# karfly/learnable-triangulation-pytorch

Hardware: AMD Instinct MI355X
Metric: multi-view samples/sec (4-view vol-softmax forward) (higher is better)
Workload: dtype bf16; 1 GPU; BASELINE config 2: volumetric-softmax forward, 4 views 384x384, 64^3 voxel cube, ResNet-152, random-init weights; per_gpu_batch=64, global_batch=64, parallelism=batch-sharded replicas x1, no data-path collective, hip_graph=True, self_launched=False

## Files before the change

include/lt_hip.h:

```cpp
#ifndef LT_HIP_H
#define LT_HIP_H

#include <stddef.h>
#include <stdint.h>

#ifdef __cplusplus
extern "C" {
#endif

#define LT_ABI_VERSION 1

enum { LT_F32 = 0, LT_BF16 = 1,
       LT_FP8 = 2  };
enum { LT_OK = 0, LT_ERR_INVALID = -1, LT_ERR_UNSUPPORTED = -2, LT_ERR_LAUNCH = -3 };

enum { LT_AGG_SUM = 0, LT_AGG_MAX = 1, LT_AGG_SOFTMAX = 2, LT_AGG_CONF = 3,
       LT_AGG_CONF_NORM = 4  };

enum {
    LT_EPI_RELU_PRE = 1,
    LT_EPI_RELU_POST = 2,
    LT_EPI_STORE_F32 = 4,
    LT_EPI_SIGMOID = 8,
    LT_EPI_RES_F32 = 64,
// ... 21 lines not shown
    int32_t dtype;
    int32_t N, D, H, W, Cin;
    int32_t Do, Ho, Wo;
    int32_t stride[3], pad[3];
    int32_t OD, OH, OW;
    int32_t out_stride[3];
    int32_t Cout, ldc;
    int32_t cout_pad, k_pad;
    int32_t nphase;
    int32_t flags;
    int32_t tile;
    int32_t stages;
    lt_conv_phase phase[LT_CONV_MAX_PHASES];
} lt_conv_desc;

int lt_conv_pack_weights(const void* weight, int32_t cout_pad, int32_t k_pad, void* packed, void* stream);
int lt_conv_pack_weights_t32(const void* weight, int32_t cout_pad, int32_t k_pad, int32_t cin, int32_t ntaps, void* packed,
                             void* stream);
int lt_conv_pack_weights32(const void* weight, int32_t cout_pad, int32_t k_pad, void* packed, void* stream);

enum { LT_TILE_AUTO = 0,
       LT_TILE_128x128 = 1, LT_TILE_128x64 = 2, LT_TILE_256x32 = 3, LT_TILE_256x16 = 4, LT_TILE_64x64 = 5,
       LT_TILE2_128x128 = 11, LT_TILE2_128x64 = 12, LT_TILE2_256x32 = 13, LT_TILE2_256x16 = 14, LT_TILE2_64x64 = 15,
       LT_TILE_HALO = 20,
       LT_TILE3_288 = 30,
       LT_TILE_DIRECT = 99  };

int lt_conv_fwd(const lt_conv_desc* desc, const void* x, const float* bias, const float* scale, const float* shift,
                const void* residual, void* y, void* stream);
typedef struct lt_conv_skip {
    const void* x;
    int32_t cin;
    const void* weight_frag;
} lt_conv_skip;
int lt_conv_skip_fwd(const lt_conv_desc* desc, const void* x, const float* bias, const float* scale, const float* shift,
                     const lt_conv_skip* skip, void* y, void* stream);
typedef struct lt_conv_cat2 {
    const void* x;
    int32_t cin, H, W, stride;
} lt_conv_cat2;
int lt_conv_cat2_fwd(const lt_conv_desc* desc, const void* x, const lt_conv_cat2* second, const float* bias, const float* scale, const float* shift,
                     const void* residual, void* y, void* stream);
int lt_conv_cout_pad(int32_t cout);
int32_t lt_conv_chunk_samples(int32_t N, int64_t per_sample);

typedef struct lt_wshape {
    int32_t nd;
    int64_t s[5];
} lt_wshape;
int lt_sel_conv_skip(int32_t dtype, const int32_t x[5], const lt_wshape* w, const int32_t skip_x[5], const lt_wshape* skip_w);
int lt_sel_halo7_col(int32_t dtype, const int32_t x[5]);
int lt_sel_halo2d_mfma(int32_t tile_rows, int32_t nphase);
int lt_sel_halo_col_mfma(int32_t kind);
int lt_sel_conv_cat2(int32_t dtype, const int32_t t2[5], const lt_wshape* w_expand, const int32_t x[5], const lt_wshape* w_down, int32_t stride_down);
int lt_sel_splitk_slices(const lt_conv_desc* d, const lt_wshape* w, int32_t transposed);
int lt_sel_bottleneck(int32_t dtype, const int32_t x[5], const lt_wshape w[3], const int32_t strides[3]);
int lt_sel_bottleneck_ds(int32_t dtype, const int32_t x[5], const lt_wshape w[3], const int32_t strides[3], const lt_wshape* w_down, int32_t stride_down);
int lt_sel_expand_reduce(int32_t dtype, const int32_t t2[5], const int32_t res[5], const lt_wshape* w_expand, const lt_wshape* w_reduce);
int lt_sel_stem_pool(int32_t dtype, const int32_t x[5], const lt_wshape* w, int32_t stride, int32_t pad, const int32_t pool[3]);
int lt_sel_pwchain(int32_t dtype, const int32_t x[5], int32_t nlayers, const lt_wshape* w);
int lt_sel_frag_layout(const lt_conv_desc* d, const lt_wshape* w, int32_t transposed, int32_t has_residual);

int lt_maxpool_fwd(int32_t dtype, const void* x, void* y, int32_t N, int32_t D, int32_t H, int32_t W, int32_t C,
                   const int32_t k[3], const int32_t s[3], const int32_t p[3], void* stream);

int lt_global_avgpool(int32_t dtype, const void* x, void* y, int32_t N, int32_t HW, int32_t C, void* stream);

int lt_nchw_to_nhwc(int32_t dtype, const float* x, void* y, int32_t N, int32_t C, int32_t HW, int32_t c_pad, void* stream);
int lt_nhwc_to_nchw_f32(int32_t dtype, const void* x, float* y, int32_t N, int32_t C, int32_t HW, int32_t ld, void* stream);

int lt_splitk_reduce(int32_t dtype, const float* partial, int32_t S, int64_t N, int64_t rows_per_sample, int32_t C, const float* bias,
                     const float* scale, const float* shift, const void* residual, void* y, int32_t flags, void* stream);

int lt_coord_volumes(const float* pos, const float* center, const float* rot, float step, int32_t B, int32_t V,
                     int32_t cmu_transfer, float* coords, void* stream);
int lt_rotate_points(const float* x, const float* rot, float* y, int64_t n, void* stream);

int lt_unproject_fwd(int32_t dtype, const void* feats, const float* proj, const float* coords, const float* conf,
                     void* out, int32_t B, int32_t NV, int32_t C, int32_t h, int32_t w, int32_t v0, int32_t v1,
                     int32_t v2, int32_t agg, void* stream);
int lt_unproject_grid_fwd(int32_t dtype, const void* feats, const float* proj, const float* pos, const float* center, const float* rot,
                          float step, int32_t cmu_transfer, float* coords_out, const float* conf, void* out, int32_t B, int32_t NV,
                          int32_t C, int32_t h, int32_t w, int32_t V, int32_t agg, void* stream);
int lt_unproject_masked_fwd(int32_t dtype, const void* feats, const float* proj, const float* coords, const float* conf, const uint8_t* view_mask,
                            void* out, int32_t B, int32_t NV, int32_t C, int32_t h, int32_t w, int32_t v0, int32_t v1, int32_t v2, int32_t agg,
                            void* stream);
int lt_unproject_grid_masked_fwd(int32_t dtype, const void* feats, const float* proj, const float* pos, const float* center, const float* rot,
                                 float step, int32_t cmu_transfer, float* coords_out, const float* conf, const uint8_t* view_mask, void* out,
                                 int32_t B, int32_t NV, int32_t C, int32_t h, int32_t w, int32_t V, int32_t agg, void* stream);
int lt_unproject_indexed_fwd(int32_t dtype, const void* feats, const float* proj, const float* coords, const float* conf, const uint8_t* view_mask,
                             const int32_t* frame_of, void* out, int32_t F, int32_t P, int32_t NV, int32_t C, int32_t h, int32_t w, int32_t v0,
                             int32_t v1, int32_t v2, int32_t agg, void* stream);
int lt_unproject_grid_indexed_fwd(int32_t dtype, const void* feats, const float* proj, const float* pos, const float* center, const float* rot,
                                  float step, int32_t cmu_transfer, float* coords_out, const float* conf, const uint8_t* view_mask,
                                  const int32_t* frame_of, void* out, int32_t F, int32_t P, int32_t NV, int32_t C, int32_t h, int32_t w, int32_t V,
                                  int32_t agg, void* stream);
enum { LT_KIND_MPII = 0, LT_KIND_COCO = 1 };
int lt_cuboid_from_keypoints(const float* keypoints_3d, int32_t B, int32_t J, int32_t kind, double cuboid_side, float* pos, float* center,
                             void* stream);

size_t lt_softargmax3d_workspace(int32_t B, int32_t J, int64_t nvox);
int lt_softargmax3d_fwd(const float* logits, const float* coords, float mult, int32_t softmax, int32_t channels_last,
                        int32_t ld, float* kp, float* probs, int32_t B, int32_t J, int64_t nvox, void* workspace,
                        void* stream);
size_t lt_softargmax3d_stats_workspace(int32_t B, int32_t J, int64_t nvox);
int lt_softargmax3d_stats_fwd(const float* logits, const float* coords, float mult, int32_t softmax, int32_t channels_last, int32_t ld,
// ... 265 lines not shown
```

learnable-triangulation-pytorch_amd/csrc/conv3d_halo_wreg.hip:

```cpp
#include "conv3d_halo.h"

namespace {

template <typename T, int CIN, int CP>
__global__ __launch_bounds__(256, (CIN == 128 ? 1 : CIN == 16 ? 4 : 2)) void conv3d_halo_wreg_kernel(const HaloArgs a) {
    constexpr int KS = 3, G = CIN / 16, NB = CP / 32;
    typedef HaloCfg<T, KS, CIN, CP, 3, 3> C;
    constexpr int TD = C::TD, TH = C::TH, TW = C::TW;
    static_assert(sizeof(T) == 2 && (NB == 1 || NB == 2 || NB == 4) && (C::CINB == 32 || C::CINB == 64 || C::CINB == 128 || C::CINB == 256),
                  "bf16; 16/32/64/128 -> 32/64/128");
    static_assert(C::SW::FB == 0, "plane-independent swizzle");
    constexpr int PLANE_B = C::HH * C::PW * C::CINB;
    constexpr int NI_H = C::HALO_BYTES / 1024;
    constexpr int FR = NB == 1 ? 2 : NB == 2 ? 4 : 8;
    constexpr bool PRE_RES = FR <= 4;
    auto wswz = [](int hh_, int hw_) -> int { return C::CINB == 256 ? ((hw_ & 7) | ((hh_ & 1) << 3)) : C::fswz(0, hh_, hw_); };

    extern __shared__ __attribute__((aligned(16))) unsigned char smem[];
    const unsigned lds0 = (unsigned)(size_t)(lptr_t)smem;
    unsigned long long zp_bits = (unsigned long long)(size_t)g_zero_page_h;
    asm volatile("" : "+s"(zp_bits));
    const void* const zero_page = (const void*)(size_t)zp_bits;

    const int t = threadIdx.x, lane = t & 63;
    const int wave = __builtin_amdgcn_readfirstlane(t >> 6);
    const int tps = a.tiles_d * a.tiles_h * a.tiles_w;
    int n, tix;
    if (a.xcd_pin) {
        const int xcd = blockIdx.x & 7, j = blockIdx.x >> 3;
        n = xcd + 8 * (j / tps);
        tix = j % tps;
    } else {
        const int nb = gridDim.x, q = nb >> 3, r = nb & 7, xcd = blockIdx.x & 7, j = blockIdx.x >> 3;
        const int lin = (xcd < r ? xcd * (q + 1) : r * (q + 1) + (xcd - r) * q) + j;
        n = lin / tps;
        tix = lin % tps;
    }
    const int w0 = (tix % a.tiles_w) * TW;
    const int h0 = ((tix / a.tiles_w) % a.tiles_h) * TH;
    const int d0 = (tix / (a.tiles_w * a.tiles_h)) * TD;
    const T* __restrict__ x = (const T*)a.x + (size_t)n * a.D * a.H * a.W * CIN;

    for (int i = wave; i < NI_H; i += 4) {
        const int q = i * 64 + lane;
        const int hv = q / C::NVV, pv = q % C::NVV;
        const int hw_ = hv % C::PW, hh_ = (hv / C::PW) % C::HH, hd_ = hv / (C::PW * C::HH);
        const int lv = pv ^ wswz(hh_, hw_);
        const int id = d0 - 1 + hd_, ih = h0 - 1 + hh_, iw = w0 - 1 + hw_;
        const bool ok = hv < C::HV && ((unsigned)id < (unsigned)a.D) & ((unsigned)ih < (unsigned)a.H) & ((unsigned)iw < (unsigned)a.W);
        const void* src = ok ? (const void*)(x + (((size_t)id * a.H + ih) * a.W + iw) * CIN + lv * C::VEC) : zero_page;
        dma16_uniform(src, lds0 + i * 1024);
    }

    const int cb = NB == 1 ? 0 : NB == 2 ? (wave & 1) : wave;
    const int p0 = NB == 1 ? wave : NB == 2 ? 2 * (wave >> 1) : 0;
    const int vl = lane & 31, hh = lane >> 5;
    unsigned lp[9][2];
#pragma unroll
    for (int i = 0; i < 2; ++i) {
        const int th = 4 * i + (vl >> 3), tw = vl & 7;
#pragma unroll
        for (int kh = 0; kh < 3; ++kh)
#pragma unroll
            for (int kw = 0; kw < 3; ++kw)
                lp[kh * 3 + kw][i] = lds0 + ((p0 * C::HH + th + kh) * C::PW + tw + kw) * C::CINB + ((hh ^ wswz(th + kh, tw + kw)) << 4);
    }
    const T* wl = (const T*)a.wfrag + ((size_t)cb * 64 + lane) * 8;
    auto load_w = [&](int u) -> V16 {
        V16 v;
        v.u = *(const uint4*)(wl + (size_t)u * NB * 64 * 8);
        return v;
    };
    constexpr int NU = 27 * G, WD = 4;
    V16 wf[WD + 1];
#pragma unroll
    for (int u = 0; u < WD; ++u) wf[u] = load_w(u);

    const size_t ldc = (size_t)a.ldc;
    const bool has_res = a.res != nullptr;
    auto out_off = [&](int f) -> size_t {
        const int td = p0 + (f >> 1), th = 4 * (f & 1) + (vl >> 3), tw = vl & 7;
        return ((((size_t)n * a.D + d0 + td) * a.H + h0 + th) * a.W + w0 + tw) * ldc + 32 * cb + 8 * hh;
    };
    uint4 rq[PRE_RES ? FR : 1][2];
    if (PRE_RES) {
#pragma unroll
        for (int f = 0; f < FR; ++f)
#pragma unroll
            for (int q = 0; q < 2; ++q)
                rq[PRE_RES ? f : 0][q] = has_res ? *(const uint4*)((const T*)a.res + out_off(f) + 16 * q) : make_uint4(0, 0, 0, 0);
    }

    f32x16 acc[FR];
#pragma unroll
    for (int f = 0; f < FR; ++f)
#pragma unroll
        for (int e = 0; e < 16; ++e) acc[f][e] = 0.f;

    asm volatile("s_waitcnt vmcnt(0)\n\ts_barrier" ::: "memory");

    V16 xa[2][FR];
    auto load_x = [&](auto uc, V16 (&dst)[FR]) {
        constexpr int u = decltype(uc)::value;
        constexpr int tap = u / G, g = u % G;
        constexpr int kd = tap / 9, khkw = tap % 9;
        const unsigned a0 = lp[khkw][0] ^ (g << 5), a1 = lp[khkw][1] ^ (g << 5);
        constexpr int HI = 3 * PLANE_B;
        const unsigned b0 = a0 + HI, b1 = a1 + HI;
        static_for<0, FR>([&](auto fc) {
            constexpr int f = decltype(fc)::value;
            constexpr int off = ((f >> 1) + kd) * PLANE_B;
            if constexpr (off + 16 <= 65536) dst[f].u = *(const uint4*)((lptr_t)(size_t)(((f & 1) ? a1 : a0) + off));
            else dst[f].u = *(const uint4*)((lptr_t)(size_t)(((f & 1) ? b1 : b0) + (off - HI)));
        });
    };
    load_x(std::integral_constant<int, 0>{}, xa[0]);
    static_for<0, NU>([&](auto uc) {
        constexpr int u = decltype(uc)::value;
        if constexpr (u + WD < NU) wf[(u + WD) % (WD + 1)] = load_w(u + WD);
        if constexpr (u + 1 < NU) load_x(std::integral_constant<int, u + 1>{}, xa[(u + 1) & 1]);
#pragma unroll
        for (int f = 0; f < FR; ++f)
            acc[f] = __builtin_amdgcn_mfma_f32_32x32x16_bf16(wf[u % (WD + 1)].h, xa[u & 1][f].h, acc[f], 0, 0, 0);
        __builtin_amdgcn_sched_barrier(0);
    });

    float esc[16], esf[16];
#pragma unroll
    for (int e = 0; e < 16; ++e) {
        const int c = 32 * cb + 16 * (e >> 3) + 8 * hh + (e & 7);
        const float bi = a.bias ? a.bias[c] : 0.f, sc = a.scale ? a.scale[c] : 1.f, sf = a.shift ? a.shift[c] : 0.f;
        esc[e] = sc; esf[e] = bi * sc + sf;
    }
    const EpiFloors fl = epi_floors(a.flags);
#pragma unroll
    for (int f = 0; f < FR; ++f) {
        const size_t oo = out_off(f);
#pragma unroll
        for (int q = 0; q < 2; ++q) {
            uint4 rv;
            if (PRE_RES) rv = rq[PRE_RES ? f : 0][q];
            else rv = has_res ? *(const uint4*)((const T*)a.res + oo + 16 * q) : make_uint4(0, 0, 0, 0);
            const unsigned rr[4] = {rv.x, rv.y, rv.z, rv.w};
            unsigned o[4];
#pragma unroll
            for (int d = 0; d < 4; ++d) {
                const int e = 8 * q + 2 * d;
                const float v0 = epi_apply(fmaf(acc[f][e], esc[e], esf[e]), fl, __uint_as_float(rr[d] << 16));
                const float v1 = epi_apply(fmaf(acc[f][e + 1], esc[e + 1], esf[e + 1]), fl, __uint_as_float(rr[d] & 0xffff0000u));
                o[d] = pack_bf16x2(v0, v1);
            }
            *(uint4*)((T*)a.y + oo + 16 * q) = make_uint4(o[0], o[1], o[2], o[3]);
        }
    }
}

__global__ void conv_pack_t32_kernel(const bf16_t* __restrict__ w, int cout_pad, int k_pad, int cin, int ntaps, bf16_t* __restrict__ out) {
    const long long g = (long long)blockIdx.x * blockDim.x + threadIdx.x;
    const int nbk = cout_pad / 32, ng = cin / 16;
    if (g >= (long long)ntaps * ng * nbk * 64) return;
    const int l = (int)(g & 63);
    long long ft = g >> 6;
    const int nb = (int)(ft % nbk); ft /= nbk;
    const int kg = (int)(ft % ng);
    const int tap = (int)(ft / ng);
    const int r = l & 31, h = l >> 5;
    const int chan = 32 * nb + 16 * (r >> 4) + 8 * ((r >> 2) & 1) + 4 * ((r >> 3) & 1) + (r & 3);
    *(uint4*)(out + g * 8) = *(const uint4*)(w + (size_t)chan * k_pad + (size_t)tap * cin + 16 * kg + 8 * h);
}

template <typename T, int CIN, int CP>
int launch_halo_wreg(const HaloArgs& a, hipStream_t s) {
    typedef HaloCfg<T, 3, CIN, CP, 3, 3> C;
    static_assert(C::HALO_BYTES <= 160 * 1024, "the halo must fit LDS");
    auto kern = conv3d_halo_wreg_kernel<T, CIN, CP>;
    LT_OPT_IN_LDS(kern, 160 * 1024);
    const long long nblk = (long long)a.N * a.tiles_d * a.tiles_h * a.tiles_w;
    hipLaunchKernelGGL(kern, dim3((unsigned)nblk), dim3(256), C::HALO_BYTES, s, a);
    LT_CHECK_LAUNCH("lt_conv_fwd(halo, weights from registers)");
    return LT_OK;
}

}

namespace lt {

int conv3d_halo_wreg_try(int cin, int cout_pad, const HaloArgs& a, hipStream_t s) {
    int rc;
    if (cin == 64 && cout_pad == 64) rc = launch_halo_wreg<bf16_t, 64, 64>(a, s);
    else if (cin == 16 && cout_pad == 32) rc = launch_halo_wreg<bf16_t, 16, 32>(a, s);
    else if (cin == 32 && cout_pad == 64) rc = launch_halo_wreg<bf16_t, 32, 64>(a, s);
    else if (cin == 128 && cout_pad == 128) rc = launch_halo_wreg<bf16_t, 128, 128>(a, s);
    else return 0;
    return rc == LT_OK ? 1 : rc;
}

}

extern "C" int lt_conv_pack_weights_t32(const void* weight, int32_t cout_pad, int32_t k_pad, int32_t cin, int32_t ntaps, void* packed,
                                        void* stream) {
    LT_REQUIRE(weight && packed, LT_ERR_INVALID, "lt_conv_pack_weights_t32: null argument");
    LT_REQUIRE(cout_pad >= 32 && cout_pad % 32 == 0 && cin >= 16 && cin % 16 == 0 && ntaps >= 1 && (long long)ntaps * cin <= k_pad && k_pad % 8 == 0,
               LT_ERR_INVALID, "lt_conv_pack_weights_t32: cout_pad %d / cin %d / ntaps %d / k_pad %d", cout_pad, cin, ntaps, k_pad);
    const long long total = (long long)ntaps * (cin / 16) * (cout_pad / 32) * 64;
    hipLaunchKernelGGL(conv_pack_t32_kernel, dim3((unsigned)((total + 255) / 256)), dim3(256), 0, (hipStream_t)stream, (const bf16_t*)weight,
                       cout_pad, k_pad, cin, ntaps, (bf16_t*)packed);
    LT_CHECK_LAUNCH("lt_conv_pack_weights_t32");
    return LT_OK;
}
```

learnable-triangulation-pytorch_amd/csrc/conv_common.h:

```cpp
#pragma once
#include "lt_common.h"

namespace lt {

typedef float f32x16 __attribute__((ext_vector_type(16)));
typedef float f32x4 __attribute__((ext_vector_type(4)));
typedef __bf16 bf16x8 __attribute__((ext_vector_type(8)));

struct PhaseArg {
    const void* w;
    const void* wfrag;
    const void* wfrag_t;
    const void* wfrag32;
    const int4* taps;
    int ntaps;
    int ood, ooh, oow;
};

struct ConvArgs {
    const void* x;
    void* y;
    const void* res;
    const float* bias;
    const float* scale;
// ... 26 lines not shown
        const lt_conv_phase& ph = d.phase[p];
        a.phase[p].w = ph.weight;
        a.phase[p].wfrag = ph.weight_frag_layout == 1 ? ph.weight_frag : nullptr;
        a.phase[p].wfrag_t = ph.weight_frag_layout == 2 ? ph.weight_frag : nullptr;
        a.phase[p].wfrag32 = ph.weight_frag_layout == 3 ? ph.weight_frag : nullptr;
        a.phase[p].taps = (const int4*)ph.taps; a.phase[p].ntaps = ph.ntaps;
        a.phase[p].ood = ph.out_off[0]; a.phase[p].ooh = ph.out_off[1]; a.phase[p].oow = ph.out_off[2];
    }
    return a;
}

inline bool halo_col_fits(long long N, int D, int H, int W) {
    if (D % 4 || H % 8 || W % 8) return false;
    const long long nblk = N * (D / 4) * (H / 8) * (W / 8), cols = N * (H / 8) * (W / 8);
    return nblk >= 1024 && nblk % 8 == 0 && D / 4 >= 2 && cols % 8 == 0 && cols >= 256;
}

inline bool halo7_col_fits(long long N, int D, int H, int W) {
    if (D % 4 || H % 8 || W % 8) return false;
    const long long cols = N * (H / 8) * (W / 8);
    return D / 4 >= 2 && cols % 8 == 0 && cols >= 256 && cols < (1ll << 31);
}

inline bool plain_pointwise(const ConvArgs& a) {
    const PhaseArg& p0 = a.phase[0];
    return p0.ntaps == 1 && a.sd == 1 && a.sh == 1 && a.sw == 1 && a.pd == 0 && a.ph == 0 && a.pw == 0 && a.osd == 1 && a.osh == 1 && a.osw == 1 &&
           p0.ood == 0 && p0.ooh == 0 && p0.oow == 0 && a.OD == a.Do && a.OH == a.Ho && a.OW == a.Wo && a.D == a.Do && a.H == a.Ho && a.W == a.Wo &&
           a.k_pad == a.Cin;
}

inline bool halo2d_fits(const ConvArgs& c, int cout_pad, int nphase) {
    if ((nphase != 1 && nphase != 4) || c.D != 1 || c.Do != 1 || c.OD != 1) return false;
    if (c.sh != 1 || c.sw != 1 || c.H != c.Ho || c.W != c.Wo || c.W % 24 || c.H % 8) return false;
    if (c.Cin != 256 || cout_pad != 256 || c.Cout != 256 || c.ldc % 8 || (c.flags & (LT_EPI_STORE_F32 | LT_EPI_SIGMOID)) || c.pd != 0) return false;
    if (nphase == 1 && (c.osh != 1 || c.osw != 1 || c.OH != c.Ho || c.OW != c.Wo || c.ph != 1 || c.pw != 1)) return false;
    if (nphase == 4 && (c.osh != 2 || c.osw != 2 || c.OH != 2 * c.Ho || c.OW != 2 * c.Wo || c.ph != 0 || c.pw != 0)) return false;
    for (int p = 0; p < nphase; ++p)
        if (c.phase[p].ntaps != (nphase == 1 ? 9 : 4) || c.phase[p].ood) return false;
    return true;
}

inline int halo2d_mfma(int tile_rows, int nphase) {
    (void)tile_rows; (void)nphase;
    return env_on("LT_H2D_MF32") ? 32 : 16;
}

inline int halo_col_mfma(int kind) {
#ifdef LT_TRACE
    return 32;
#endif
    return kind == 2 || env_on("LT_HALO_COL_MF32") ? 32 : 16;
}

union V16 {
    uint4 u;
    f32x4 f;
    bf16x8 h;
};

template <typename T, int MF> struct Mma;
template <> struct Mma<float, 32> {
    typedef f32x16 acc_t;
    static __device__ __forceinline__ void run(acc_t& c, const V16& a, const V16& b) {
#pragma unroll
        for (int e = 0; e < 4; ++e) c = __builtin_amdgcn_mfma_f32_32x32x2f32(a.f[e], b.f[e], c, 0, 0, 0);
    }
};
template <> struct Mma<float, 16> {
    typedef f32x4 acc_t;
    static __device__ __forceinline__ void run(acc_t& c, const V16& a, const V16& b) {
#pragma unroll
        for (int e = 0; e < 4; ++e) c = __builtin_amdgcn_mfma_f32_16x16x4f32(a.f[e], b.f[e], c, 0, 0, 0);
    }
};
template <> struct Mma<bf16_t, 32> {
    typedef f32x16 acc_t;
    static __device__ __forceinline__ void run(acc_t& c, const V16& a, const V16& b) {
        c = __builtin_amdgcn_mfma_f32_32x32x16_bf16(a.h, b.h, c, 0, 0, 0);
    }
};
template <> struct Mma<bf16_t, 16> {
    typedef f32x4 acc_t;
    static __device__ __forceinline__ void run(acc_t& c, const V16& a, const V16& b) {
        c = __builtin_amdgcn_mfma_f32_16x16x32_bf16(a.h, b.h, c, 0, 0, 0);
    }
};

union V16Q {
    uint4 u;
    long q[2];
};
template <> struct Mma<fp8_t, 32> {
    typedef f32x16 acc_t;
    static __device__ __forceinline__ void run(acc_t& c, const V16& a, const V16& b) {
        V16Q qa, qb;
        qa.u = a.u; qb.u = b.u;
        c = __builtin_amdgcn_mfma_f32_32x32x16_fp8_fp8(qa.q[0], qb.q[0], c, 0, 0, 0);
        c = __builtin_amdgcn_mfma_f32_32x32x16_fp8_fp8(qa.q[1], qb.q[1], c, 0, 0, 0);
    }
};
template <> struct Mma<fp8_t, 16> {
    typedef f32x4 acc_t;
    static __device__ __forceinline__ void run(acc_t& c, const V16& a, const V16& b) {
        V16Q qa, qb;
        qa.u = a.u; qb.u = b.u;
        c = __builtin_amdgcn_mfma_f32_16x16x32_fp8_fp8(qa.q[0], qb.q[0], c, 0, 0, 0);
// ... 28 lines not shown
```

learnable-triangulation-pytorch_amd/csrc/select.hip:

```cpp
#include "conv_common.h"

using namespace lt;

namespace {

bool wshape_is(const lt_wshape* w, int nd, int64_t s0, int64_t s1, int64_t s2, int64_t s3, int64_t s4 = 0) {
    const int64_t s[5] = {s0, s1, s2, s3, s4};
    if (w->nd != nd) return false;
    for (int i = 0; i < nd; ++i)
        if (w->s[i] != s[i]) return false;
    return true;
}

bool pointwise(const lt_wshape* w) {
    for (int i = 2; i < w->nd; ++i)
        if (w->s[i] != 1) return false;
    return true;
}

}

extern "C" int lt_sel_conv_skip(int32_t dtype, const int32_t x[5], const lt_wshape* w, const int32_t skip_x[5], const lt_wshape* skip_w) {
    if (dtype != LT_BF16 || env_on("LT_NO_CONV_SKIP") || env_on("LT_HALO_NO_COL") || env_on("LT_HALO_NO_PERSIST") || env_on("LT_CONV_NO_HALO")) return 0;
    if (!wshape_is(w, 5, 32, 32, 3, 3, 3) || !wshape_is(skip_w, 5, 32, 16, 1, 1, 1)) return 0;
    const int N = x[0], D = x[1], H = x[2], W = x[3];
    if (x[4] != 32 || skip_x[0] != N || skip_x[1] != D || skip_x[2] != H || skip_x[3] != W || skip_x[4] != 16) return 0;
    const int nc = lt_conv_chunk_samples(N, (long long)D * H * W * 32);
    if (nc < 1) return 0;
    return halo_col_fits(nc, D, H, W) && halo_col_fits(N - (N - 1) / nc * nc, D, H, W);
}

extern "C" int lt_sel_halo7_col(int32_t dtype, const int32_t x[5]) {
    if (dtype != LT_BF16 || x[4] != 32 || env_on("LT_HALO_NO_COL7")) return 0;
    return halo7_col_fits(x[0], x[1], x[2], x[3]);
}

extern "C" int lt_sel_halo2d_mfma(int32_t tile_rows, int32_t nphase) {
    if ((tile_rows != 8 && tile_rows != 4) || (nphase != 1 && nphase != 4) || (tile_rows == 4 && nphase == 4)) return 0;
    return halo2d_mfma(tile_rows, nphase);
}

extern "C" int lt_sel_halo_col_mfma(int32_t kind) { return kind < 0 || kind > 2 ? 0 : halo_col_mfma(kind); }

extern "C" int lt_sel_conv_cat2(int32_t dtype, const int32_t t2[5], const lt_wshape* we, const int32_t x[5], const lt_wshape* wd, int32_t s) {
    if (dtype != LT_BF16 || env_on("LT_NO_CONV_CAT2") || env_on("LT_CONV_NO_V7") || env_on("LT_CONV_NO_V3")) return 0;
    const int N = t2[0], Ho = t2[2], Wo = t2[3], P = t2[4];
    if (t2[1] != 1 || we->nd != 4 || wd->nd != 4 || !pointwise(we) || !pointwise(wd)) return 0;
    const long long Cc = we->s[0], Cin2 = wd->s[1];
    if (we->s[1] != P || wd->s[0] != Cc || (s != 1 && s != 2) || x[0] != N || x[1] != 1 || x[2] != Ho * s || x[3] != Wo * s || x[4] != Cin2) return 0;
    if (P % 32 || Cin2 % 32 || (P + Cin2) % 64 || Cc % 256 || (P & (P - 1))) return 0;
    const long long tiles = (((long long)N * Ho * Wo + 287) / 288) * (Cc / 256);
    if (tiles < 200 && !env_on("LT_CAT2_ANY_SIZE")) return 0;
    return (long long)N * Ho * Wo * Cc < (1ll << 31) && (long long)N * x[2] * x[3] * Cin2 < (1ll << 31);
}

extern "C" int lt_sel_splitk_slices(const lt_conv_desc* d, const lt_wshape* w, int32_t transposed) {
    if (d->dtype != LT_BF16 || transposed || (d->flags & (LT_EPI_STORE_F32 | LT_EPI_SIGMOID)) || env_on("LT_CONV_NO_SPLITK")) return 1;
    if (w->nd != 5 || w->s[2] != 3 || w->s[3] != 3 || w->s[4] != 3) return 1;
    for (int i = 0; i < 3; ++i)
        if (d->stride[i] != 1 || d->pad[i] != 1) return 1;
    if (d->Cin < 128 || d->Cin % 64 || d->Cout % 4 || d->Cout != d->cout_pad || d->D * d->H * d->W > 512) return 1;
    const long long rows = (long long)d->N * d->Do * d->Ho * d->Wo;
    const int bm = rows >= 8192 ? 128 : 64;
    const long long tiles = ((rows + bm - 1) / bm) * (d->cout_pad / bm);
    const long long S = 256 / tiles;
    return S > 8 ? 8 : S < 1 ? 1 : (int)S;
}

extern "C" int lt_sel_bottleneck(int32_t dtype, const int32_t x[5], const lt_wshape w[3], const int32_t strides[3]) {
    if (dtype != LT_BF16 || env_on("LT_NO_BNECK")) return 0;
    if (x[1] != 1 || strides[0] != 1 || strides[1] != 1 || strides[2] != 1) return 0;
    const int C = x[4];
    const int64_t P = w[0].s[0];
    if (!((C == 256 && P == 64) || (C == 512 && P == 128))) return 0;
    if (!wshape_is(&w[0], 4, P, C, 1, 1) || !wshape_is(&w[1], 4, P, P, 3, 3) || !wshape_is(&w[2], 4, C, P, 1, 1)) return 0;
    return x[2] % 8 == 0 && x[3] % 16 == 0 && (long long)x[0] * x[2] * x[3] * C < (1ll << 31);
}

extern "C" int lt_sel_bottleneck_ds(int32_t dtype, const int32_t x[5], const lt_wshape w[3], const int32_t strides[3], const lt_wshape* wd, int32_t sd) {
    if (dtype != LT_BF16 || env_on("LT_NO_BNECK") || env_on("LT_NO_BNECK_DS")) return 0;
    if (x[1] != 1 || strides[0] != 1 || strides[1] != 1 || strides[2] != 1 || sd != 1) return 0;
    if (x[4] != 64 || !wshape_is(&w[0], 4, 64, 64, 1, 1) || !wshape_is(&w[1], 4, 64, 64, 3, 3) || !wshape_is(&w[2], 4, 256, 64, 1, 1) ||
        !wshape_is(wd, 4, 256, 64, 1, 1))
        return 0;
    return x[2] % 8 == 0 && x[3] % 16 == 0 && (long long)x[0] * x[2] * x[3] * 256 < (1ll << 31);
}

extern "C" int lt_sel_expand_reduce(int32_t dtype, const int32_t t2[5], const int32_t res[5], const lt_wshape* we, const lt_wshape* wr) {
    if (dtype != LT_BF16 || env_on("LT_NO_XR")) return 0;
    if (t2[1] != 1 || res[1] != 1 || t2[0] != res[0] || t2[2] != res[2] || t2[3] != res[3] || res[4] != 1024 || t2[4] != 256) return 0;
    if ((long long)t2[0] * t2[2] * t2[3] < 36 * 96 && !env_on("LT_XR_ANY_SIZE")) return 0;
    return wshape_is(we, 4, 1024, 256, 1, 1) && wshape_is(wr, 4, 256, 1024, 1, 1);
}

extern "C" int lt_sel_stem_pool(int32_t dtype, const int32_t x[5], const lt_wshape* w, int32_t stride, int32_t pad, const int32_t pool[3]) {
// ... 33 lines not shown
```

learnable-triangulation-pytorch_amd/lt_hip.py:

```python
import ctypes as C
import os

import torch

HERE = os.path.dirname(os.path.abspath(__file__))
LIB_PATH = os.environ.get("LT_HIP_LIB") or os.path.join(HERE, "lib", "liblt_hip.so")

LT_F32, LT_BF16, LT_FP8 = 0, 1, 2
AGG = {"sum": 0, "max": 1, "softmax": 2, "conf": 3, "conf_norm": 4}
LT_MODEL_ALG, LT_MODEL_RANSAC = 1, 2
LT_KIND_MPII, LT_KIND_COCO = 0, 1
KIND = {"mpii": LT_KIND_MPII, "coco": LT_KIND_COCO}
EPI_RELU_PRE, EPI_RELU_POST, EPI_STORE_F32, EPI_SIGMOID = 1, 2, 4, 8
EPI_RES_F32 = 64
BN_FROZEN = 32
BN_Y_BF16 = 128
ACT_BF16 = 256
TILE_AUTO, TILE_128x128, TILE_128x64, TILE_256x32, TILE_256x16, TILE_64x64, TILE_DIRECT = 0, 1, 2, 3, 4, 5, 99
TILE2_128x128, TILE2_128x64, TILE2_256x32, TILE2_256x16, TILE2_64x64 = 11, 12, 13, 14, 15
TILE_HALO = 20
TILE3_288 = 30
MAX_PHASES = 8

vp, i32, i64, f32, f64 = C.c_void_p, C.c_int32, C.c_int64, C.c_float, C.c_double
# ... 63 lines not shown

class NamedTensor(C.Structure):
    _fields_ = [("name", C.c_char_p), ("data", vp), ("ndim", i32), ("shape", C.c_int64 * 5)]


class VolPlanConfig(C.Structure):
    _fields_ = [("dtype", i32), ("num_layers", i32), ("style_caffe", i32), ("num_joints", i32), ("B", i32), ("NV", i32), ("H", i32), ("W", i32),
                ("volume_size", i32), ("cuboid_side", C.c_double), ("volume_multiplier", C.c_double), ("volume_softmax", i32), ("aggregation", i32),
                ("transfer_cmu_to_human36m", i32), ("use_graph", i32)]


class AlgPlanConfig(C.Structure):
    _fields_ = [("model", i32), ("dtype", i32), ("num_layers", i32), ("style_caffe", i32), ("num_joints", i32), ("B", i32), ("NV", i32), ("H", i32),
                ("W", i32), ("use_confidences", i32), ("heatmap_softmax", i32), ("heatmap_multiplier", C.c_double), ("direct_optimization", i32),
                ("reprojection_error_epsilon", C.c_double), ("use_graph", i32)]


class CascadePlanConfig(C.Structure):
    _fields_ = [("alg", AlgPlanConfig), ("vol", VolPlanConfig), ("kind", i32)]


class PlanInfo(C.Structure):
    _fields_ = [("launches", i32), ("heatmap_h", i32), ("heatmap_w", i32), ("flops", C.c_double), ("bytes_allocated", C.c_int64),
                ("n_expand_reduce", i32), ("n_bottleneck", i32), ("n_bottleneck_ds", i32), ("n_conv_cat2", i32), ("n_conv2d_halo", i32), ("n_pwchain", i32),
                ("n_stem_pool", i32), ("n_splitk", i32), ("n_conv_skip", i32), ("graph_captured", i32), ("logits", vp), ("logits_planar", i32)]


SIGNATURES = {
    "lt_plan_create_vol": (C.c_int, [C.POINTER(VolPlanConfig), C.POINTER(NamedTensor), i32, C.POINTER(vp)]),
    "lt_plan_forward_vol": (C.c_int, [vp, vp, vp, vp, vp, vp, vp, vp, vp, vp, vp, vp, vp]),
    "lt_plan_create_vol_multi": (C.c_int, [C.POINTER(VolPlanConfig), i32, C.POINTER(NamedTensor), i32, C.POINTER(vp)]),
    "lt_plan_forward_vol_multi": (C.c_int, [vp, vp, vp, vp, vp, vp, vp, vp, vp, vp, vp, vp, vp, vp]),
    "lt_plan_create_alg": (C.c_int, [C.POINTER(AlgPlanConfig), C.POINTER(NamedTensor), i32, C.POINTER(vp)]),
    "lt_plan_forward_alg": (C.c_int, [vp, vp, vp, vp, vp, vp, vp, vp]),
    "lt_plan_create_cascade": (C.c_int, [C.POINTER(CascadePlanConfig), C.POINTER(NamedTensor), i32, C.POINTER(NamedTensor), i32, C.POINTER(vp)]),
    "lt_plan_forward_cascade": (C.c_int, [vp, vp, vp, vp, vp, vp, vp, vp, vp, vp, vp, vp, vp, vp]),
    "lt_plan_set_view_mask": (C.c_int, [vp, vp]),
    "lt_plan_set_keypoint_stats": (C.c_int, [vp, vp, vp]),
    "lt_plan_set_alg_keypoint_stats": (C.c_int, [vp, vp, vp, vp, vp, vp]),
    "lt_plan_info": (C.c_int, [vp, C.POINTER(PlanInfo)]),
    "lt_plan_destroy": (None, [vp]),
    "lt_last_error": (C.c_char_p, []),
    "lt_abi_version": (C.c_int, []),
    "lt_device_info": (C.c_int, [C.POINTER(C.c_int), C.POINTER(C.c_int), C.c_char_p, C.c_int]),
    "lt_conv_fwd": (C.c_int, [C.POINTER(ConvDesc), vp, vp, vp, vp, vp, vp, vp]),
    "lt_conv_skip_fwd": (C.c_int, [C.POINTER(ConvDesc), vp, vp, vp, vp, C.POINTER(ConvSkip), vp, vp]),
    "lt_conv_cat2_fwd": (C.c_int, [C.POINTER(ConvDesc), vp, C.POINTER(ConvCat2), vp, vp, vp, vp, vp, vp]),
    "lt_conv_cout_pad": (C.c_int, [i32]),
    "lt_conv_chunk_samples": (i32, [i32, i64]),
    "lt_sel_conv_skip": (C.c_int, [i32, i32 * 5, C.POINTER(WShape), i32 * 5, C.POINTER(WShape)]),
    "lt_sel_halo7_col": (C.c_int, [i32, i32 * 5]),
    "lt_sel_halo2d_mfma": (C.c_int, [i32, i32]),
    "lt_sel_halo_col_mfma": (C.c_int, [i32]),
    "lt_sel_conv_cat2": (C.c_int, [i32, i32 * 5, C.POINTER(WShape), i32 * 5, C.POINTER(WShape), i32]),
    "lt_sel_splitk_slices": (C.c_int, [C.POINTER(ConvDesc), C.POINTER(WShape), i32]),
    "lt_sel_bottleneck": (C.c_int, [i32, i32 * 5, WShape * 3, i32 * 3]),
    "lt_sel_bottleneck_ds": (C.c_int, [i32, i32 * 5, WShape * 3, i32 * 3, C.POINTER(WShape), i32]),
    "lt_sel_expand_reduce": (C.c_int, [i32, i32 * 5, i32 * 5, C.POINTER(WShape), C.POINTER(WShape)]),
    "lt_sel_stem_pool": (C.c_int, [i32, i32 * 5, C.POINTER(WShape), i32, i32, i32 * 3]),
    "lt_sel_pwchain": (C.c_int, [i32, i32 * 5, i32, C.POINTER(WShape)]),
    "lt_sel_frag_layout": (C.c_int, [C.POINTER(ConvDesc), C.POINTER(WShape), i32, i32]),
    "lt_conv_pack_weights": (C.c_int, [vp, i32, i32, vp, vp]),
    "lt_conv_pack_weights_t32": (C.c_int, [vp, i32, i32, i32, i32, vp, vp]),
    "lt_conv_pack_weights32": (C.c_int, [vp, i32, i32, vp, vp]),
    "lt_pwchain_fwd": (C.c_int, [C.POINTER(PwChainDesc), vp, vp, vp]),
    "lt_stem_pool_fwd": (C.c_int, [C.POINTER(StemDesc), vp, vp, vp]),
    "lt_bottleneck_fwd": (C.c_int, [C.POINTER(BneckDesc), vp, vp, vp]),
    "lt_bottleneck_ds_fwd": (C.c_int, [C.POINTER(BneckDsDesc), vp, vp, vp]),
    "lt_expand_reduce_fwd": (C.c_int, [C.POINTER(XrDesc), vp, vp, vp, vp, vp]),
    "lt_stem_packed_bytes": (C.c_size_t, []),
    "lt_stem_pack_weights": (C.c_int, [vp, i32, vp, vp]),
    "lt_maxpool_fwd": (C.c_int, [i32, vp, vp, i32, i32, i32, i32, i32, i32 * 3, i32 * 3, i32 * 3, vp]),
    "lt_global_avgpool": (C.c_int, [i32, vp, vp, i32, i32, i32, vp]),
    "lt_nchw_to_nhwc": (C.c_int, [i32, vp, vp, i32, i32, i32, i32, vp]),
    "lt_nhwc_to_nchw_f32": (C.c_int, [i32, vp, vp, i32, i32, i32, i32, vp]),
    "lt_coord_volumes": (C.c_int, [vp, vp, vp, f32, i32, i32, i32, vp, vp]),
    "lt_rotate_points": (C.c_int, [vp, vp, vp, i64, vp]),
    "lt_unproject_fwd": (C.c_int, [i32, vp, vp, vp, vp, vp, i32, i32, i32, i32, i32, i32, i32, i32, i32, vp]),
    "lt_unproject_grid_fwd": (C.c_int, [i32, vp, vp, vp, vp, vp, f32, i32, vp, vp, vp, i32, i32, i32, i32, i32, i32, i32, vp]),
    "lt_unproject_masked_fwd": (C.c_int, [i32, vp, vp, vp, vp, vp, vp, i32, i32, i32, i32, i32, i32, i32, i32, i32, vp]),
    "lt_unproject_grid_masked_fwd": (C.c_int, [i32, vp, vp, vp, vp, vp, f32, i32, vp, vp, vp, vp, i32, i32, i32, i32, i32, i32, i32, vp]),
    "lt_unproject_indexed_fwd": (C.c_int, [i32, vp, vp, vp, vp, vp, vp, vp, i32, i32, i32, i32, i32, i32, i32, i32, i32, i32, vp]),
    "lt_unproject_grid_indexed_fwd": (C.c_int, [i32, vp, vp, vp, vp, vp, f32, i32, vp, vp, vp, vp, vp, i32, i32, i32, i32, i32, i32, i32, i32, vp]),
    "lt_cuboid_from_keypoints": (C.c_int, [vp, i32, i32, i32, C.c_double, vp, vp, vp]),
    "lt_softargmax3d_workspace": (C.c_size_t, [i32, i32, i64]),
    "lt_softargmax3d_fwd": (C.c_int, [vp, vp, f32, i32, i32, i32, vp, vp, i32, i32, i64, vp, vp]),
    "lt_softargmax3d_stats_workspace": (C.c_size_t, [i32, i32, i64]),
    "lt_softargmax3d_stats_fwd": (C.c_int, [vp, vp, f32, i32, i32, i32, vp, vp, vp, vp, i32, i32, i64, vp, vp]),
    "lt_softargmax2d_fwd": (C.c_int, [vp, f32, i32, vp, vp, i32, i32, i32, vp]),
    "lt_softargmax2d_stats_fwd": (C.c_int, [vp, f32, i32, vp, vp, vp, vp, i32, i32, i32, vp]),
    "lt_triangulate_dlt": (C.c_int, [vp, vp, vp, vp, i32, i32, i32, vp]),
    "lt_alg_tail_fwd": (C.c_int, [vp, vp, i32, vp, f32, f32, vp, vp, vp, i32, i32, i32, vp]),
    "lt_alg_tail_masked_fwd": (C.c_int, [vp, vp, i32, vp, f32, f32, vp, vp, vp, vp, i32, i32, i32, vp]),
    "lt_alg_tail_stats_fwd": (C.c_int, [vp, vp, i32, vp, f32, f32, vp, vp, vp, vp, vp, vp, vp, vp, i32, i32, i32, vp]),
    "lt_triangulate_dlt_stats": (C.c_int, [vp, vp, vp, vp, vp, vp, vp, vp, i32, i32, i32, vp]),
    "lt_heatmap_argmax_nchw_f32": (C.c_int, [vp, i32, vp, vp, vp, i32, i32, i32, i32, i32, i32, vp]),
    "lt_triangulate_ransac": (C.c_int, [vp, vp, vp, i32, C.c_double, i32, vp, vp, i32, i32, i32, vp]),
    "lt_crop_resize_u8": (C.c_int, [vp, i64, vp, vp, i32, i32, i32, vp, vp, vp]),
    "lt_undistort_crop_resize_u8": (C.c_int, [vp, i64, vp, vp, vp, i64, i32, i32, i32, vp, vp, vp]),
    "lt_bn_act_fwd": (C.c_int, [vp, vp, vp, vp, vp, vp, vp, vp, i64, i32, f32, i32, vp]),
    "lt_bn_act_bwd_workspace": (C.c_size_t, [i64, i32]),
    "lt_bn_act_bwd": (C.c_int, [vp, vp, vp, vp, vp, vp, vp, vp, vp, vp, vp, vp, i32, i64, i32, f32, i32, vp, vp]),
    "lt_act_bwd": (C.c_int, [vp, vp, vp, vp, vp, i32, i64, i32, vp]),
    "lt_channel_sum_workspace": (C.c_size_t, [i64, i32]),
    "lt_channel_sum": (C.c_int, [vp, i64, i32, vp, i32, vp, vp]),
    "lt_channel_sum_dt": (C.c_int, [i32, vp, i64, i32, vp, i32, vp, vp]),
# ... 162 lines not shown
```

Measured before the change: 1511 samples/s.

## Use 16x16x32 MFMA variant in weight-register 3D halo conv kernel

Measured after the change: 1512 samples/s (median of 2 runs). No clear change (+0.1%).

```diff
diff --git a/include/lt_hip.h b/include/lt_hip.h
--- a/include/lt_hip.h
+++ b/include/lt_hip.h
@@ -97,6 +97,7 @@
 int lt_sel_halo7_col(int32_t dtype, const int32_t x[5]);
 int lt_sel_halo2d_mfma(int32_t tile_rows, int32_t nphase);
 int lt_sel_halo_col_mfma(int32_t kind);
+int lt_sel_halo_wreg_mfma(int32_t cin, int32_t cout_pad);
 int lt_sel_conv_cat2(int32_t dtype, const int32_t t2[5], const lt_wshape* w_expand, const int32_t x[5], const lt_wshape* w_down, int32_t stride_down);
 int lt_sel_splitk_slices(const lt_conv_desc* d, const lt_wshape* w, int32_t transposed);
 int lt_sel_bottleneck(int32_t dtype, const int32_t x[5], const lt_wshape w[3], const int32_t strides[3]);
diff --git a/learnable-triangulation-pytorch_amd/csrc/conv3d_halo_wreg.hip b/learnable-triangulation-pytorch_amd/csrc/conv3d_halo_wreg.hip
--- a/learnable-triangulation-pytorch_amd/csrc/conv3d_halo_wreg.hip
+++ b/learnable-triangulation-pytorch_amd/csrc/conv3d_halo_wreg.hip
@@ -2,19 +2,23 @@
 
 namespace {
 
-template <typename T, int CIN, int CP>
+template <typename T, int CIN, int CP, int MF>
 __global__ __launch_bounds__(256, (CIN == 128 ? 1 : CIN == 16 ? 4 : 2)) void conv3d_halo_wreg_kernel(const HaloArgs a) {
     constexpr int KS = 3, G = CIN / 16, NB = CP / 32;
     typedef HaloCfg<T, KS, CIN, CP, 3, 3> C;
     constexpr int TD = C::TD, TH = C::TH, TW = C::TW;
     static_assert(sizeof(T) == 2 && (NB == 1 || NB == 2 || NB == 4) && (C::CINB == 32 || C::CINB == 64 || C::CINB == 128 || C::CINB == 256),
                   "bf16; 16/32/64/128 -> 32/64/128");
+    static_assert(MF == 32 || (MF == 16 && G % 2 == 0 && NB >= 2), "32x32x16, or 16x16x32 with whole K blocks of 32 channels");
     static_assert(C::SW::FB == 0, "plane-independent swizzle");
     constexpr int PLANE_B = C::HH * C::PW * C::CINB;
     constexpr int NI_H = C::HALO_BYTES / 1024;
     constexpr int FR = NB == 1 ? 2 : NB == 2 ? 4 : 8;
     constexpr bool PRE_RES = FR <= 4;
-    auto wswz = [](int hh_, int hw_) -> int { return C::CINB == 256 ? ((hw_ & 7) | ((hh_ & 1) << 3)) : C::fswz(0, hh_, hw_); };
+    auto wswz = [](int hh_, int hw_) -> int {
+        return MF == 16 ? (C::CINB == 256 ? ((hh_ & 1) | ((hw_ & 7) << 1)) : (((hh_ & 1) | (((hw_ >> 1) & 3) << 1)) & (C::NVV - 1)))
+                        : C::CINB == 256 ? ((hw_ & 7) | ((hh_ & 1) << 3)) : C::fswz(0, hh_, hw_);
+    };
 
     extern __shared__ __attribute__((aligned(16))) unsigned char smem[];
     const unsigned lds0 = (unsigned)(size_t)(lptr_t)smem;
@@ -54,103 +58,170 @@
 
     const int cb = NB == 1 ? 0 : NB == 2 ? (wave & 1) : wave;
     const int p0 = NB == 1 ? wave : NB == 2 ? 2 * (wave >> 1) : 0;
-    const int vl = lane & 31, hh = lane >> 5;
+    const int vl = lane & (MF - 1), hh = lane / MF;
+    const int vrow = MF == 32 ? vl >> 3 : vl & 1, vcol = MF == 32 ? vl & 7 : vl >> 1;
     unsigned lp[9][2];
 #pragma unroll
     for (int i = 0; i < 2; ++i) {
-        const int th = 4 * i + (vl >> 3), tw = vl & 7;
+        const int th = 4 * i + vrow, tw = vcol;
 #pragma unroll
         for (int kh = 0; kh < 3; ++kh)
 #pragma unroll
             for (int kw = 0; kw < 3; ++kw)
                 lp[kh * 3 + kw][i] = lds0 + ((p0 * C::HH + th + kh) * C::PW + tw + kw) * C::CINB + ((hh ^ wswz(th + kh, tw + kw)) << 4);
     }
-    const T* wl = (const T*)a.wfrag + ((size_t)cb * 64 + lane) * 8;
+    const int wlane = MF == 32 ? lane : (lane >> 5) * NB * 64 + 32 * (hh & 1) + ((vl & 7) | (vl >> 3) << 4);
+    const T* wl = (const T*)a.wfrag + ((size_t)cb * 64 + wlane) * 8;
     auto load_w = [&](int u) -> V16 {
         V16 v;
-        v.u = *(const uint4*)(wl + (size_t)u * NB * 64 * 8);
+        if constexpr (MF == 32) v.u = *(const uint4*)(wl + (size_t)u * NB * 64 * 8);
+        else v.u = *(const uint4*)(wl + (size_t)(u >> 1) * 2 * NB * 64 * 8 + (u & 1) * 8 * 8);
         return v;
     };
-    constexpr int NU = 27 * G, WD = 4;
-    V16 wf[WD + 1];
+    constexpr int NU = 27 * G, WD = 4, NS = MF == 32 ? WD + 1 : WD + 2;
+    V16 wf[NS];
 #pragma unroll
     for (int u = 0; u < WD; ++u) wf[u] = load_w(u);
 
+    constexpr int NF = FR * 32 / MF, NQ = MF / 16;
     const size_t ldc = (size_t)a.ldc;
     const bool has_res = a.res != nullptr;
     auto out_off = [&](int f) -> size_t {
-        const int td = p0 + (f >> 1), th = 4 * (f & 1) + (vl >> 3), tw = vl & 7;
+        const int td = p0 + (MF == 32 ? f >> 1 : f >> 2), th = (MF == 32 ? 4 * (f & 1) : 2 * (f & 3)) + vrow, tw = vcol;
         return ((((size_t)n * a.D + d0 + td) * a.H + h0 + th) * a.W + w0 + tw) * ldc + 32 * cb + 8 * hh;
     };
-    uint4 rq[PRE_RES ? FR : 1][2];
+    uint4 rq[PRE_RES ? NF : 1][NQ];
     if (PRE_RES) {
 #pragma unroll
-        for (int f = 0; f < FR; ++f)
-#pragma unroll
-            for (int q = 0; q < 2; ++q)
+        for (int f = 0; f < NF; ++f)
+#pragma unroll
+            for (int q = 0; q < NQ; ++q)
                 rq[PRE_RES ? f : 0][q] = has_res ? *(const uint4*)((const T*)a.res + out_off(f) + 16 * q) : make_uint4(0, 0, 0, 0);
     }
-
-    f32x16 acc[FR];
-#pragma unroll
-    for (int f = 0; f < FR; ++f)
-#pragma unroll
-        for (int e = 0; e < 16; ++e) acc[f][e] = 0.f;
-
-    asm volatile("s_waitcnt vmcnt(0)\n\ts_barrier" ::: "memory");
-
-    V16 xa[2][FR];
-    auto load_x = [&](auto uc, V16 (&dst)[FR]) {
-        constexpr int u = decltype(uc)::value;
-        constexpr int tap = u / G, g = u % G;
-        constexpr int kd = tap / 9, khkw = tap % 9;
-        const unsigned a0 = lp[khkw][0] ^ (g << 5), a1 = lp[khkw][1] ^ (g << 5);
-        constexpr int HI = 3 * PLANE_B;
-        const unsigned b0 = a0 + HI, b1 = a1 + HI;
-        static_for<0, FR>([&](auto fc) {
-            constexpr int f = decltype(fc)::value;
-            constexpr int off = ((f >> 1) + kd) * PLANE_B;
-            if constexpr (off + 16 <= 65536) dst[f].u = *(const uint4*)((lptr_t)(size_t)(((f & 1) ? a1 : a0) + off));
-            else dst[f].u = *(const uint4*)((lptr_t)(size_t)(((f & 1) ? b1 : b0) + (off - HI)));
+    auto residual = [&](int f, int q, size_t oo) -> uint4 {
+        if (PRE_RES) return rq[PRE_RES ? f : 0][q];
+        return has_res ? *(const uint4*)((const T*)a.res + oo + 16 * q) : make_uint4(0, 0, 0, 0);
+    };
+    constexpr int NE = MF / 2;
+    float esc[NE], esf[NE];
+    auto load_consts = [&]() {
+#pragma unroll
+        for (int e = 0; e < NE; ++e) {
+            const int c = MF == 32 ? 32 * cb + 16 * (e >> 3) + 8 * hh + (e & 7) : 32 * cb + 8 * hh + e;
+            const float bi = a.bias ? a.bias[c] : 0.f, sc = a.scale ? a.scale[c] : 1.f, sf = a.shift ? a.shift[c] : 0.f;
+            esc[e] = sc; esf[e] = bi * sc + sf;
+        }
+    };
+    const EpiFloors fl = epi_floors(a.flags);
+    constexpr int HI = 3 * PLANE_B;
+
+    if constexpr (MF == 16) {
+        f32x4 acc[2][FR][2];
+#pragma unroll
+        for (int f = 0; f < 2 * FR; ++f)
+#pragma unroll
+            for (int e = 0; e < 4; ++e) acc[f / FR][f % FR][0][e] = acc[f / FR][f % FR][1][e] = 0.f;
+
+        asm volatile("s_waitcnt vmcnt(0)\n\ts_barrier" ::: "memory");
+
+        constexpr int NKB = 27 * (G / 2), NST = 2 * NKB, WB = WD / 2;
+        V16 xa[2][FR];
+        auto load_x = [&](auto tc, V16 (&dst)[FR]) {
+            constexpr int t_ = decltype(tc)::value, kb = t_ / 2, hf = t_ % 2, tap = kb / (G / 2), m = kb % (G / 2);
+            constexpr int kd = tap / 9, khkw = tap % 9;
+            const unsigned a0 = lp[khkw][0] ^ (m << 6), a1 = lp[khkw][1] ^ (m << 6);
+            const unsigned b0 = a0 + HI, b1 = a1 + HI;
+            static_for<0, FR>([&](auto fc) {
+                constexpr int f = hf * FR + decltype(fc)::value;
+                constexpr int off = ((f >> 2) + kd) * PLANE_B + 2 * (f & 1) * C::PW * C::CINB;
+                if constexpr (off + 16 <= 65536) dst[f % FR].u = *(const uint4*)((lptr_t)(size_t)(((f & 2) ? a1 : a0) + off));
+                else dst[f % FR].u = *(const uint4*)((lptr_t)(size_t)(((f & 2) ? b1 : b0) + (off - HI)));
+            });
+        };
+        load_x(std::integral_constant<int, 0>{}, xa[0]);
+        static_for<0, NST>([&](auto tc) {
+            constexpr int t_ = decltype(tc)::value, kb = t_ / 2, hf = t_ % 2;
+            if constexpr (hf == 0 && kb + WB < NKB) {
+#pragma unroll
+                for (int s = 0; s < 2; ++s) wf[(2 * (kb + WB) + s) % NS] = load_w(2 * (kb + WB) + s);
+            }
+            if constexpr (t_ + 1 < NST) load_x(std::integral_constant<int, t_ + 1>{}, xa[(t_ + 1) % 2]);
+#pragma unroll
+            for (int f = 0; f < FR; ++f)
+#pragma unroll
+                for (int s = 0; s < 2; ++s)
+                    acc[hf][f][s] = __builtin_amdgcn_mfma_f32_16x16x32_bf16(wf[(2 * kb + s) % NS].h, xa[t_ % 2][f].h, acc[hf][f][s], 0, 0, 0);
+            __builtin_amdgcn_sched_barrier(0);
         });
-    };
-    load_x(std::integral_constant<int, 0>{}, xa[0]);
-    static_for<0, NU>([&](auto uc) {
-        constexpr int u = decltype(uc)::value;
-        if constexpr (u + WD < NU) wf[(u + WD) % (WD + 1)] = load_w(u + WD);
-        if constexpr (u + 1 < NU) load_x(std::integral_constant<int, u + 1>{}, xa[(u + 1) & 1]);
-#pragma unroll
-        for (int f = 0; f < FR; ++f)
-            acc[f] = __builtin_amdgcn_mfma_f32_32x32x16_bf16(wf[u % (WD + 1)].h, xa[u & 1][f].h, acc[f], 0, 0, 0);
-        __builtin_amdgcn_sched_barrier(0);
-    });
-
-    float esc[16], esf[16];
-#pragma unroll
-    for (int e = 0; e < 16; ++e) {
-        const int c = 32 * cb + 16 * (e >> 3) + 8 * hh + (e & 7);
-        const float bi = a.bias ? a.bias[c] : 0.f, sc = a.scale ? a.scale[c] : 1.f, sf = a.shift ? a.shift[c] : 0.f;
-        esc[e] = sc; esf[e] = bi * sc + sf;
-    }
-    const EpiFloors fl = epi_floors(a.flags);
-#pragma unroll
-    for (int f = 0; f < FR; ++f) {
-        const size_t oo = out_off(f);
-#pragma unroll
-        for (int q = 0; q < 2; ++q) {
-            uint4 rv;
-            if (PRE_RES) rv = rq[PRE_RES ? f : 0][q];
-            else rv = has_res ? *(const uint4*)((const T*)a.res + oo + 16 * q) : make_uint4(0, 0, 0, 0);
+
+        load_consts();
+#pragma unroll
+        for (int f = 0; f < NF; ++f) {
+            const size_t oo = out_off(f);
+            const uint4 rv = residual(f, 0, oo);
             const unsigned rr[4] = {rv.x, rv.y, rv.z, rv.w};
             unsigned o[4];
 #pragma unroll
             for (int d = 0; d < 4; ++d) {
-                const int e = 8 * q + 2 * d;
-                const float v0 = epi_apply(fmaf(acc[f][e], esc[e], esf[e]), fl, __uint_as_float(rr[d] << 16));
-                const float v1 = epi_apply(fmaf(acc[f][e + 1], esc[e + 1], esf[e + 1]), fl, __uint_as_float(rr[d] & 0xffff0000u));
+                const int e = 2 * d, s = d >> 1, r = e & 3;
+                const float v0 = epi_apply(fmaf(acc[f / FR][f % FR][s][r], esc[e], esf[e]), fl, __uint_as_float(rr[d] << 16));
+                const float v1 = epi_apply(fmaf(acc[f / FR][f % FR][s][r + 1], esc[e + 1], esf[e + 1]), fl, __uint_as_float(rr[d] & 0xffff0000u));
                 o[d] = pack_bf16x2(v0, v1);
             }
-            *(uint4*)((T*)a.y + oo + 16 * q) = make_uint4(o[0], o[1], o[2], o[3]);
+            *(uint4*)((T*)a.y + oo) = make_uint4(o[0], o[1], o[2], o[3]);
+        }
+    } else {
+        f32x16 acc[FR];
+#pragma unroll
+        for (int f = 0; f < FR; ++f)
+#pragma unroll
+            for (int e = 0; e < 16; ++e) acc[f][e] = 0.f;
+
+        asm volatile("s_waitcnt vmcnt(0)\n\ts_barrier" ::: "memory");
+
+        V16 xa[2][FR];
+        auto load_x = [&](auto uc, V16 (&dst)[FR]) {
+            constexpr int u = decltype(uc)::value;
+            constexpr int tap = u / G, g = u % G;
+            constexpr int kd = tap / 9, khkw = tap % 9;
+            const unsigned a0 = lp[khkw][0] ^ (g << 5), a1 = lp[khkw][1] ^ (g << 5);
+            const unsigned b0 = a0 + HI, b1 = a1 + HI;
+            static_for<0, FR>([&](auto fc) {
+                constexpr int f = decltype(fc)::value;
+                constexpr int off = ((f >> 1) + kd) * PLANE_B;
+                if constexpr (off + 16 <= 65536) dst[f].u = *(const uint4*)((lptr_t)(size_t)(((f & 1) ? a1 : a0) + off));
+                else dst[f].u = *(const uint4*)((lptr_t)(size_t)(((f & 1) ? b1 : b0) + (off - HI)));
+            });
+        };
+        load_x(std::integral_constant<int, 0>{}, xa[0]);
+        static_for<0, NU>([&](auto uc) {
+            constexpr int u = decltype(uc)::value;
+            if constexpr (u + WD < NU) wf[(u + WD) % NS] = load_w(u + WD);
+            if constexpr (u + 1 < NU) load_x(std::integral_constant<int, u + 1>{}, xa[(u + 1) & 1]);
+#pragma unroll
+            for (int f = 0; f < FR; ++f)
+                acc[f] = __builtin_amdgcn_mfma_f32_32x32x16_bf16(wf[u % NS].h, xa[u & 1][f].h, acc[f], 0, 0, 0);
+            __builtin_amdgcn_sched_barrier(0);
+        });
+
+        load_consts();
+#pragma unroll
+        for (int f = 0; f < FR; ++f) {
+            const size_t oo = out_off(f);
+#pragma unroll
+            for (int q = 0; q < 2; ++q) {
+                const uint4 rv = residual(f, q, oo);
+                const unsigned rr[4] = {rv.x, rv.y, rv.z, rv.w};
+                unsigned o[4];
+#pragma unroll
+                for (int d = 0; d < 4; ++d) {
+                    const int e = 8 * q + 2 * d;
+                    const float v0 = epi_apply(fmaf(acc[f][e], esc[e], esf[e]), fl, __uint_as_float(rr[d] << 16));
+                    const float v1 = epi_apply(fmaf(acc[f][e + 1], esc[e + 1], esf[e + 1]), fl, __uint_as_float(rr[d] & 0xffff0000u));
+                    o[d] = pack_bf16x2(v0, v1);
+                }
+                *(uint4*)((T*)a.y + oo + 16 * q) = make_uint4(o[0], o[1], o[2], o[3]);
+            }
         }
     }
 }
@@ -169,11 +240,11 @@
     *(uint4*)(out + g * 8) = *(const uint4*)(w + (size_t)chan * k_pad + (size_t)tap * cin + 16 * kg + 8 * h);
 }
 
-template <typename T, int CIN, int CP>
+template <typename T, int CIN, int CP, int MF>
 int launch_halo_wreg(const HaloArgs& a, hipStream_t s) {
     typedef HaloCfg<T, 3, CIN, CP, 3, 3> C;
     static_assert(C::HALO_BYTES <= 160 * 1024, "the halo must fit LDS");
-    auto kern = conv3d_halo_wreg_kernel<T, CIN, CP>;
+    auto kern = conv3d_halo_wreg_kernel<T, CIN, CP, MF>;
     LT_OPT_IN_LDS(kern, 160 * 1024);
     const long long nblk = (long long)a.N * a.tiles_d * a.tiles_h * a.tiles_w;
     hipLaunchKernelGGL(kern, dim3((unsigned)nblk), dim3(256), C::HALO_BYTES, s, a);
@@ -186,11 +257,12 @@
 namespace lt {
 
 int conv3d_halo_wreg_try(int cin, int cout_pad, const HaloArgs& a, hipStream_t s) {
+    const bool mf16 = halo_wreg_mfma(cin, cout_pad) == 16;
     int rc;
-    if (cin == 64 && cout_pad == 64) rc = launch_halo_wreg<bf16_t, 64, 64>(a, s);
-    else if (cin == 16 && cout_pad == 32) rc = launch_halo_wreg<bf16_t, 16, 32>(a, s);
-    else if (cin == 32 && cout_pad == 64) rc = launch_halo_wreg<bf16_t, 32, 64>(a, s);
-    else if (cin == 128 && cout_pad == 128) rc = launch_halo_wreg<bf16_t, 128, 128>(a, s);
+    if (cin == 64 && cout_pad == 64) rc = mf16 ? launch_halo_wreg<bf16_t, 64, 64, 16>(a, s) : launch_halo_wreg<bf16_t, 64, 64, 32>(a, s);
+    else if (cin == 16 && cout_pad == 32) rc = launch_halo_wreg<bf16_t, 16, 32, 32>(a, s);
+    else if (cin == 32 && cout_pad == 64) rc = mf16 ? launch_halo_wreg<bf16_t, 32, 64, 16>(a, s) : launch_halo_wreg<bf16_t, 32, 64, 32>(a, s);
+    else if (cin == 128 && cout_pad == 128) rc = mf16 ? launch_halo_wreg<bf16_t, 128, 128, 16>(a, s) : launch_halo_wreg<bf16_t, 128, 128, 32>(a, s);
     else return 0;
     return rc == LT_OK ? 1 : rc;
 }
diff --git a/learnable-triangulation-pytorch_amd/csrc/conv_common.h b/learnable-triangulation-pytorch_amd/csrc/conv_common.h
--- a/learnable-triangulation-pytorch_amd/csrc/conv_common.h
+++ b/learnable-triangulation-pytorch_amd/csrc/conv_common.h
@@ -102,6 +102,12 @@
     return kind == 2 || env_on("LT_HALO_COL_MF32") ? 32 : 16;
 }
 
+inline int halo_wreg_mfma(int cin, int cout_pad) {
+    if (cin == 16 && cout_pad == 32) return 32;
+    if (!((cin == 64 && cout_pad == 64) || (cin == 32 && cout_pad == 64) || (cin == 128 && cout_pad == 128))) return 0;
+    return env_on("LT_HALO_WREG_MF32") ? 32 : 16;
+}
+
 union V16 {
     uint4 u;
     f32x4 f;
diff --git a/learnable-triangulation-pytorch_amd/csrc/select.hip b/learnable-triangulation-pytorch_amd/csrc/select.hip
--- a/learnable-triangulation-pytorch_amd/csrc/select.hip
+++ b/learnable-triangulation-pytorch_amd/csrc/select.hip
@@ -41,6 +41,8 @@
 }
 
 extern "C" int lt_sel_halo_col_mfma(int32_t kind) { return kind < 0 || kind > 2 ? 0 : halo_col_mfma(kind); }
+
+extern "C" int lt_sel_halo_wreg_mfma(int32_t cin, int32_t cout_pad) { return halo_wreg_mfma(cin, cout_pad); }
 
 extern "C" int lt_sel_conv_cat2(int32_t dtype, const int32_t t2[5], const lt_wshape* we, const int32_t x[5], const lt_wshape* wd, int32_t s) {
     if (dtype != LT_BF16 || env_on("LT_NO_CONV_CAT2") || env_on("LT_CONV_NO_V7") || env_on("LT_CONV_NO_V3")) return 0;
diff --git a/learnable-triangulation-pytorch_amd/lt_hip.py b/learnable-triangulation-pytorch_amd/lt_hip.py
--- a/learnable-triangulation-pytorch_amd/lt_hip.py
+++ b/learnable-triangulation-pytorch_amd/lt_hip.py
@@ -139,6 +139,7 @@
     "lt_sel_halo7_col": (C.c_int, [i32, i32 * 5]),
     "lt_sel_halo2d_mfma": (C.c_int, [i32, i32]),
     "lt_sel_halo_col_mfma": (C.c_int, [i32]),
+    "lt_sel_halo_wreg_mfma": (C.c_int, [i32, i32]),
     "lt_sel_conv_cat2": (C.c_int, [i32, i32 * 5, C.POINTER(WShape), i32 * 5, C.POINTER(WShape), i32]),
     "lt_sel_splitk_slices": (C.c_int, [C.POINTER(ConvDesc), C.POINTER(WShape), i32]),
     "lt_sel_bottleneck": (C.c_int, [i32, i32 * 5, WShape * 3, i32 * 3]),
```
